# hangelwen/miR-PREFeR

Hardware: AMD Instinct MI355X
Metric: precursor windows folded+filtered/sec (L=300) (higher is better)
Workload: dtype int16/int32 (energies in 0.01 kcal/mol)

## Files before the change

mir-prefer_amd/csrc/fold_lds_kernel.hip:

```cpp
#include <algorithm>
#include "fold_lds_common.h"
#include "fold_ctl.h"
#ifndef MIRP_CPERIOD0
#define MIRP_CPERIOD0 0
#endif
#ifndef MIRP_CPERIOD1
#define MIRP_CPERIOD1 64
#endif
#define CPOOL_ROUNDS 4

namespace mirp {

template <int MODEL, bool SPARSE, int NT = LNT>
__global__ void __launch_bounds__(NT, 4) fold_lds_kernel(
    const FoldParams* __restrict__ P, const unsigned char* __restrict__ seqs, const long long* __restrict__ offs, const int* __restrict__ win_lens,
    int n_work, int win_base, int span, short* __restrict__ slabs, size_t slab_shorts, int* __restrict__ win_state,
    unsigned int* __restrict__ work_counter, int* __restrict__ fallback_list,
    unsigned int* __restrict__ fallback_count, int max_lines, int ss_stride, MirpFoldLine* __restrict__ out_lines, char* __restrict__ out_ss,
    int* __restrict__ out_nlines, int* __restrict__ out_mfe, int* __restrict__ out_status, int light_clocks_arg, long long* __restrict__ dbg_cycles_arg,
    const int* __restrict__ todo_list, const unsigned int* __restrict__ todo_count, int* __restrict__ dense_list, unsigned int* __restrict__ dense_count) {
#include "fold_lds_kernel_body.h"
}

template <int MODEL, bool SPARSE, int NT>
__device__ __forceinline__ void fold_lds_body(

    const FoldParams* __restrict__ P, const unsigned char* __restrict__ seqs, const long long* __restrict__ offs, const int* __restrict__ win_lens,
    int n_work, int win_base, int span, short* __restrict__ slabs, size_t slab_shorts, int* __restrict__ win_state,
    unsigned int* __restrict__ work_counter, int* __restrict__ fallback_list,
    unsigned int* __restrict__ fallback_count, int max_lines, int ss_stride, MirpFoldLine* __restrict__ out_lines, char* __restrict__ out_ss,
    int* __restrict__ out_nlines, int* __restrict__ out_mfe, int* __restrict__ out_status, int light_clocks_arg, long long* __restrict__ dbg_cycles_arg,
    const int* __restrict__ todo_list, const unsigned int* __restrict__ todo_count, int* __restrict__ dense_list, unsigned int* __restrict__ dense_count) {
#include "fold_lds_kernel_body.h"
}
#ifndef MIRP_FILL_TWO_ATTR
#define MIRP_FILL_TWO_ATTR __attribute__((amdgpu_num_vgpr(56)))
#endif
template <>
__global__ void MIRP_FILL_TWO_ATTR __launch_bounds__(LNT2, 4) fold_lds_kernel<0, true, LNT2>(

    const FoldParams* __restrict__ P, const unsigned char* __restrict__ seqs, const long long* __restrict__ offs, const int* __restrict__ win_lens,
    int n_work, int win_base, int span, short* __restrict__ slabs, size_t slab_shorts, int* __restrict__ win_state,
    unsigned int* __restrict__ work_counter, int* __restrict__ fallback_list,
    unsigned int* __restrict__ fallback_count, int max_lines, int ss_stride, MirpFoldLine* __restrict__ out_lines, char* __restrict__ out_ss,
    int* __restrict__ out_nlines, int* __restrict__ out_mfe, int* __restrict__ out_status, int light_clocks_arg, long long* __restrict__ dbg_cycles_arg,
    const int* __restrict__ todo_list, const unsigned int* __restrict__ todo_count, int* __restrict__ dense_list, unsigned int* __restrict__ dense_count) {
    fold_lds_body<0, true, LNT2>(P, seqs, offs, win_lens, n_work, win_base, span, slabs, slab_shorts, win_state, work_counter, fallback_list, fallback_count, max_lines, ss_stride, out_lines, out_ss, out_nlines, out_mfe, out_status, light_clocks_arg, dbg_cycles_arg, todo_list, todo_count, dense_list, dense_count);
}

#ifndef ENT
#define ENT 256
#endif
#ifndef MIRP_EPI_WGS
#define MIRP_EPI_WGS 8
#endif
__global__ void __launch_bounds__(ENT, MIRP_EPI_WGS) fold_lds_epilogue_kernel(
    const FoldParams* __restrict__ P, const unsigned char* __restrict__ seqs, const long long* __restrict__ offs, const int* __restrict__ win_lens,
    int n_work, int span, const short* __restrict__ slabs, size_t slab_shorts, const int* __restrict__ win_state, unsigned int* __restrict__ work_counter,
    int max_lines, int ss_stride, MirpFoldLine* __restrict__ out_lines, char* __restrict__ out_ss, int* __restrict__ out_nlines,
    int* __restrict__ out_mfe, int* __restrict__ out_status) {
    extern __shared__ __align__(16) unsigned char smem[];
    const int nc = LCAP + 8;
    int* f3 = (int*)smem;
    int* starts = f3 + nc;
    int* lens = starts + max_lines;
    int* btstk = lens + max_lines;
    int* misc = btstk + (ENT / 64) * 3 * BT_STACK;
    int* off = misc + 16;
    short* spec = (short*)(off + LDMAX + 2);
    unsigned char* S = (unsigned char*)(spec + 3 * nc);
    unsigned char* seq = S + nc;
    char* btbuf = (char*)(seq + nc);
    EpiTables* EP = (EpiTables*)(smem + ((((size_t)(btbuf - (char*)smem) + (ENT / 64) * nc) + 15) & ~(size_t)15));
    short* xtab = (short*)(EP + 1);
    unsigned char* pq2 = (unsigned char*)(xtab + XTAB_N);
    short* ppart = (short*)(pq2 + nc);
    const int tid = threadIdx.x;
    fill_epi_tables(EP, P, tid, ENT);
    fill_ext_table(xtab, P, tid, ENT);
    __syncthreads();
    EPI_INIT();
    for (;;) {
        if (tid == 0) misc[0] = (int)atomicAdd(work_counter, 1u);
        __syncthreads();
        const int win = misc[0];
        __syncthreads();
        if (win >= n_work) break;
        if (win_state[win] == 1) {
            const long long o0 = offs[win];
            const int n = win_lens ? win_lens[win] : (int)(offs[win + 1] - o0);
            const int D = (span - 1 < n - 1) ? span - 1 : n - 1;
            for (int x = tid; x <= n + 1; x += ENT) {
                unsigned char ch = 0;
                if (x >= 1 && x <= n) {
                    ch = seqs[o0 + x - 1];
                    if (ch >= 'a' && ch <= 'z') ch -= 32;
                    if (ch == 'T') ch = 'U';
                }
                seq[x] = ch;
                S[x] = ch == 'A' ? 1 : ch == 'C' ? 2 : ch == 'G' ? 3 : ch == 'U' ? 4 : 0;
            }
            if (tid < ARCH_RB) off[tid] = arch_rowblk_off(tid, n, span);
            __syncthreads();
            if (tid == 0) { S[0] = S[n]; S[n + 1] = S[1]; }
            for (int x = tid + 1; x <= n; x += ENT) pq2[x] = (unsigned char)((S[x] * 6 + (x < n ? (int)S[x + 1] : 5)) * 2);
            special_hairpins(P, seq, n, spec, nc, tid, ENT);
            __syncthreads();
            WinCtx X;
            X.P = P; X.S = S; X.seq = seq; X.f3 = f3; X.spec = spec; X.ldspec = nc; X.n = n; X.D = D; X.E = EP; X.xtab = xtab; X.pq2 = pq2; X.pp = ppart;
            LTab TB;
            TB.carch = slabs + (size_t)win * 3 * slab_shorts; TB.fml = TB.carch + slab_shorts; TB.off = off;
            TB.tb = reinterpret_cast<const unsigned short*>(TB.carch + 2 * slab_shorts);
            fold_epilogue<LTab, ENT>(X, TB, span, f3, starts, lens, btbuf, nc, btstk, misc + 8, win, max_lines, ss_stride, out_lines, out_ss, out_nlines,
                                    out_mfe, out_status);
        }
        __syncthreads();
    }
    EPI_FLUSH();
}

struct LTab185 {
    static constexpr bool kTiled = true;
    const short* carch;
    const short* fml;
    const unsigned short* tb;
    const int* off;
    int n, D, Dm;
    __device__ __forceinline__ int at(int d, int i) const { return off[(i - 1) >> 3] + ((i - 1) & 7) + 8 * (d - 4); }
    __device__ __forceinline__ int C(int i, int j) const {
        const int d = j - i;
        if (d <= TURN || d > D || i < 1 || j > n) return V_INF;
        const int v = carch[at(d, i)];
        return v == I16_INF ? V_INF : v;
    }
    __device__ __forceinline__ int Mm(int i, int j) const {
        const int d = j - i;
        if (d <= TURN || d > Dm || i < 1 || j > n) return V_INF;
        const int v = (unsigned short)fml[at(d, i)];
        return v == 65535 ? V_INF : v - FML_BIAS;
    }
    __device__ __forceinline__ int TB(int i, int j) const { return tb[at(j - i, i)]; }
};

#ifndef MIRP_EPI185_WGS
#define MIRP_EPI185_WGS 8
#endif
__global__ void __launch_bounds__(ENT, MIRP_EPI185_WGS) fold185_lds_epilogue_kernel(
    const FoldParams* __restrict__ P, const unsigned char* __restrict__ seqs, const long long* __restrict__ offs, const int* __restrict__ win_lens,
    int n_work, int span, const short* __restrict__ slabs, size_t slab_shorts, const int* __restrict__ win_state, unsigned int* __restrict__ work_counter,
    int max_lines, int ss_stride, MirpFoldLine* __restrict__ out_lines, char* __restrict__ out_ss, int* __restrict__ out_nlines,
    int* __restrict__ out_mfe, int* __restrict__ out_status) {
    extern __shared__ __align__(16) unsigned char smem[];
    const int nc = LCAP + 8;
    int* f3 = (int*)smem;
    int* starts = f3 + nc + 8;
    int* lens = starts + max_lines;
    int* btstk = lens + max_lines;
    int* red = btstk + (ENT / 64) * 3 * V_BT_STACK;
    int* misc = red + ENT / 64 + 8;
    int* off = misc + 4;
    short* tetra = (short*)(off + LDMAX + 2);
    unsigned char* S = (unsigned char*)(tetra + nc);
    unsigned char* seq = S + nc;
    char* btbuf = (char*)(seq + nc);
    short* dg = (short*)(smem + ((((size_t)(btbuf - (char*)smem) + (ENT / 64) * (nc + 8)) + 15) & ~(size_t)15));
    const int tid = threadIdx.x;
    if (tid < 40) { dg[tid] = (short)P->dangle5[tid / 5][tid % 5]; dg[40 + tid] = (short)P->dangle3[tid / 5][tid % 5]; }
    __syncthreads();
    EPI_INIT();
    for (;;) {
        if (tid == 0) misc[0] = (int)atomicAdd(work_counter, 1u);
        __syncthreads();
        const int win = misc[0];
        __syncthreads();
        if (win >= n_work) break;
        if (win_state[win] == 1) {
            const long long o0 = offs[win];
            const int n = win_lens ? win_lens[win] : (int)(offs[win + 1] - o0);
            for (int x = tid; x <= n + 1; x += ENT) {
                unsigned char ch = 0;
                if (x >= 1 && x <= n) {
                    ch = seqs[o0 + x - 1];
                    if (ch >= 'a' && ch <= 'z') ch -= 32;
                    if (ch == 'T') ch = 'U';
                }
                seq[x] = ch;
// ... 136 lines not shown
```

mir-prefer_amd/csrc/fold_lds_kernel_body.h:

```cpp
    extern __shared__ __align__(16) unsigned char smem[];
    constexpr bool TWO = NT != LNT;
    static_assert(NT == LNT || NT == LNT2, "workgroup size");
    constexpr int NW = NT / 64;
    constexpr LdsLayout LY = lds_layout<MODEL, SPARSE, TWO>();
#ifdef MIRP_DIAG
    const bool light = light_clocks_arg != 0;
    long long* const dbg_cycles = dbg_cycles_arg;
#else
    constexpr bool light = false;
    constexpr long long* dbg_cycles = nullptr;
    (void)light_clocks_arg; (void)dbg_cycles_arg;
#endif
    constexpr int DMLR = MODEL ? 5 : 3;
#define ENT_OUTER(mmo, mm1) ((unsigned)(((mmo) & 1023) | (((mm1) & 1023) << 10)))
    const int tau_s = __builtin_amdgcn_readfirstlane(P->TerminalAU);
    constexpr int GEN_WD = 5;
    long long tA = 0, tB = 0, tS = 0, tE = 0, t0 = 0;
    long long tR = 0, nR = 0, nB = 0;
    long long wB = 0, wA1 = 0, wA2 = 0, wW = 0, wt = 0;
    unsigned short* fml = (unsigned short*)(smem + LY.fml);
    unsigned short* cring = (unsigned short*)(smem + LY.aux);
    short* dmlring = (short*)(cring + CRING_ROWS * CSTR);
    int* acc = (int*)(dmlring + DMLR * LCAP);
    constexpr int NACC = SPARSE ? 6 : 5;
// ... 208 lines not shown
                }
                const int k0 = (NW - 1 - wave) * 64 + lane;
#pragma unroll
                for (int r = 0; r < A2_PRE; r++) {
                    const int k = k0 + r * NT;
                    if (k < lim) {
                        int i; bool ok;
                        (void)a2_entry(k, i, ok);
                        const unsigned sum = a2g[r] + (unsigned)poolB[k];
                        if (ok && sum < 65535u) atomicMin(&mdec[i], (int)sum - 2 * FML_BIAS);
                    }
                }
                for (int k = k0 + A2_PRE * NT; k < lim; k += NT) {
                    int i; bool ok;
                    const unsigned g = fml_g[a2_entry(k, i, ok)];
                    const unsigned sum = g + (unsigned)poolB[k];
                    if (ok && sum < 65535u) atomicMin(&mdec[i], (int)sum - 2 * FML_BIAS);
                }
                asm volatile("s_waitcnt lgkmcnt(0)" : "+v"(pnv) : : "memory");
                { const int pn = __builtin_amdgcn_readfirstlane(pnv); sp_snap = pn < pool_cap ? pn : pool_cap; }
            };
            auto splits_sparse185 = [&]() {
                const int lim = sp_snap;
                int pnv;
                {
                    const unsigned pa = (unsigned)(size_t)(__attribute__((address_space(3))) int*)&misc[3];
                    asm volatile("ds_read_b32 %0, %1" : "=v"(pnv) : "v"(pa) : "memory");
                }
                for (int k = (NW - 1 - wave) * 64 + lane; k < lim; k += NT) {
                    const unsigned lo = poolA[k], hi = poolB32[k];
                    const int p = (int)(lo & 511u), q = (int)((lo >> 9) & 511u);
                    const int valb = (int)(hi & 0xffffu), e5 = -(int)((hi >> 16) & 255u), e3 = -(int)(hi >> 24);
                    const int i0 = q - d, t0 = p - 1 - i0;
                    const int oA0 = 7 - 4 * n + (__mul24(t0, 2 * n + 1 - t0) >> 1) + ((t0 - 4 + (n & 1)) >> 1) + i0;
                    const int oA1 = oA0 - tri_len_any(t0 - 1, n);
                    const int oB1 = oA1 - tri_len_any(t0 - 2, n) + 1;
                    const bool c0 = i0 >= 1, c1 = i0 >= 0 && q + 1 <= n;
                    const bool vA0 = c0 && t0 >= TURN + 1, vA1 = c0 && t0 - 1 >= TURN + 1, vB0 = c1 && t0 - 1 >= TURN + 1, vB1 = c1 && t0 - 2 >= TURN + 1;
                    const int a0 = fml[vA0 ? oA0 : 1], a1 = fml[vA1 ? oA1 : 1], b0 = fml[vB0 ? oA1 + 1 : 1], b1 = fml[vB1 ? oB1 : 1];
                    int best0 = INF, best1 = INF;
                    if (vA0 && a0 != 65535) best0 = a0 + valb;
                    if (vA1 && a1 != 65535) { const int v = a1 + valb + e5; best0 = v < best0 ? v : best0; }
                    if (vB0 && b0 != 65535) best1 = b0 + valb + e3;
                    if (vB1 && b1 != 65535) { const int v = b1 + valb + e5 + e3; best1 = v < best1 ? v : best1; }
                    if (best0 < INF) atomicMin(&mdec[i0], best0 - 2 * FML_BIAS);
                    if (best1 < INF) atomicMin(&mdec[i0 + 1], best1 - 2 * FML_BIAS);
                }
                asm volatile("s_waitcnt lgkmcnt(0)" : "+v"(pnv) : : "memory");
                { const int pn = __builtin_amdgcn_readfirstlane(pnv); sp_snap = pn < pool_cap ? pn : pool_cap; }
            };
            auto splits_dense = [&]() {
                const int npair = (ncell + 1) >> 1;
                const int ncpad = (npair + 63) & ~63;
                if (ncpad != sp_ncpad) {
                    sp_ncpad = ncpad;
                    sp_nsub = (NT / ncpad) & ~1;
                    sp_pair = tid % ncpad;
                    sp_sub = __builtin_amdgcn_readfirstlane(tid / ncpad);
                    const int t0 = 4 + sp_sub, u0 = d - t0 - 1, s1 = sp_nsub;
                    sp_so1 = __builtin_amdgcn_readfirstlane(2 * tri_off(t0, n));
                    sp_si1 = __builtin_amdgcn_readfirstlane(2 * (tri_off(t0 + s1, n) - tri_off(t0, n)));
                    sp_so2 = __builtin_amdgcn_readfirstlane(2 * (tri_off(u0, n) + t0 + 1 - ((t0 & 1) ? 0 : 1)));
                    sp_si2 = __builtin_amdgcn_readfirstlane(2 * (tri_off(u0 - s1, n) - tri_off(u0, n) + s1));
                } else {
                    const int uprev = d - 1 - (4 + sp_sub) - 1;
                    sp_so2 += 2 * tri_len_any(uprev, n);
                    sp_si2 += 2 * sp_nsub;
                }
                const int nsub = sp_nsub, pair = sp_pair, sub = sp_sub;
                if (sub < nsub) {
                    const int i = 2 * pair + 1;
                    const int s1 = nsub;
                    int t = 4 + sub;
                    const int odd = t & 1;
                    int so1 = sp_so1, so2 = sp_so2, si1 = sp_si1, si2 = sp_si2;
                    const int sss = 2 * s1 * s1;
                    us2 bu = {65535, 65535};
                    typedef const __attribute__((address_space(3))) unsigned* lds_cu32;
                    const unsigned fb0 = (unsigned)(size_t)(lds_cu32)reinterpret_cast<const unsigned*>(fml + i);
                    unsigned va = fb0 + (unsigned)so1, vb = fb0 + (unsigned)so2;
#define MIRP_SSTEP() do { va += (unsigned)si1; vb += (unsigned)si2; asm volatile("s_sub_i32 %0, %0, %2\n\ts_sub_i32 %1, %1, %2" : "+s"(si1), "+s"(si2) : "s"(sss) : "scc"); } while (0)
#define MIRP_LDA() (*(lds_cu32)(va))
#define MIRP_LDB(o) (*(lds_cu32)(vb + (o)))
                    auto group = [&](auto ODD, auto KK) {
                        constexpr bool kOdd = decltype(ODD)::value;
                        constexpr int K = decltype(KK)::value;
                        unsigned a[K], b[K], c[K];
#pragma unroll
                        for (int k = 0; k < K; k++) {
                            a[k] = MIRP_LDA(); b[k] = MIRP_LDB(0);
                            if (!kOdd) c[k] = MIRP_LDB(4);
                            MIRP_SSTEP();
                        }
                        us2 e[K];
#pragma unroll
                        for (int k = 0; k < K; k++) {
                            const unsigned bw = kOdd ? b[k] : __builtin_amdgcn_alignbit(c[k], b[k], 16);
                            us2 av, bv;
                            __builtin_memcpy(&av, &a[k], 4); __builtin_memcpy(&bv, &bw, 4);
                            e[k] = __builtin_elementwise_add_sat(av, bv);
                        }
#pragma unroll
                        for (int w = 1; w < K; w *= 2)
#pragma unroll
                            for (int k = 0; k + w < K; k += 2 * w) e[k] = __builtin_elementwise_min(e[k], e[k + w]);
                        bu = __builtin_elementwise_min(bu, e[0]);
                        t += K * s1;
                    };
                    auto relax = [&](auto ODD) {
                        while (t + 7 * s1 <= d - 5) group(ODD, std::integral_constant<int, 8>{});
                        if (t + 3 * s1 <= d - 5) group(ODD, std::integral_constant<int, 4>{});
                        if (t + s1 <= d - 5) group(ODD, std::integral_constant<int, 2>{});
                        if (t <= d - 5) group(ODD, std::integral_constant<int, 1>{});
                    };
                    if (odd) relax(std::true_type{}); else relax(std::false_type{});
#undef MIRP_SSTEP
#undef MIRP_LDA
#undef MIRP_LDB
                    const unsigned r0 = bu[0], r1 = bu[1];
                    if (i <= ncell && r0 < 65535u) atomicMin(&mdec[i], (int)r0 - 2 * FML_BIAS);
                    if (i + 1 <= ncell && r1 < 65535u) atomicMin(&mdec[i + 1], (int)r1 - 2 * FML_BIAS);
                }
            };
            const bool swap_order = !SPARSE && (wave & 1);
            auto splits = [&]() { if constexpr (SPARSE && MODEL != 0) splits_sparse185(); else if constexpr (TWO) splits_sparse2(); else if constexpr (SPARSE) splits_sparse(); else splits_dense(); };
            if (swap_order) splits();
            if constexpr (TWO) a2_prefetch();
            if (dbg_cycles && lane == 0 && !light) wt = clock64();
            if (d >= 6 && d <= D) {
                const list_t* clist = list + (d % 3) * LSEG;
                const bool mix = d - 2 - (TURN + 1) >= MAXLOOP && d + 1 <= D;
                const int ncp = a1_ncp;
                const int done = a1_done;
                const int rem = ncp - done;
                const int nblk = (rem + 63) >> 6;
                int ncp2;
                if (lc_have) { asm volatile("s_waitcnt lgkmcnt(0)" : "+v"(lc_pre) : : "memory"); ncp2 = __builtin_amdgcn_readfirstlane(lc_pre); }
                else ncp2 = __builtin_amdgcn_readfirstlane(lcnt[(d + 1) % 6]);
                a1_ncp = ncp2;
                const int room = nblk * 64 - rem;
                const int take2 = mix ? (room < ncp2 ? room : ncp2) : 0;
                a1_done = take2;
                unsigned* ckey2 = reinterpret_cast<unsigned*>(acc + MIRP_CK(d + 1) * LCAP);
                unsigned aent = 0;
                {
                    const int ka = lane - (64 - room);
                    if (ka >= 0 && ka < take2) aent = list[((d + 1) % 3) * LSEG + ka];
                }
#define MIRP_XROWS15 9, 7
#define MIRP_XROWS8 8
#define MIRP_XROWS9 10
                A1 a;
                a.P = P; a.T = &T; a.S = S; a.cring = cring; a.pax = pax; a.qbr = qbr; a.code4 = code4; a.n = n;
#pragma nounroll
                for (int pass = 0; pass < (TWO ? 2 : 1); pass++) {
                const int role = TWO ? (wave < 4 ? wave + 8 * pass : wave < 6 ? (pass ? wave : wave + 10) : (pass ? wave : wave + 6))
                                     : wave < 4 ? wave : wave < 6 ? wave + 10 : wave < 12 ? wave + 2 : wave - 8;
                for (int blk = 0; blk < nblk; blk++) {
                    {
                        int r0 = d - 2, um = d - 2 - (TURN + 1) < MAXLOOP ? d - 2 - (TURN + 1) : MAXLOOP;
                        asm volatile("" : "+s"(r0), "+s"(um));
                        a.r0 = r0; a.um = um;
                        a.rowtab = P->ring_rowoff[r0 & 31];
                    }
                    const int k = blk * 64 + lane;
                    const bool own = k < rem, ahead = !own && aent != 0;
                    const bool act = own || ahead;
                    const unsigned ent = own ? clist[done + k] : ahead ? aent : (1u | (1u << 9));
                    const int i = ent & 511, type = (ent >> 9) & 7, j = i + d + (ahead ? 1 : 0);
                    a.cring = cring + (ahead ? CSTR : 0);
                    unsigned* ck = ahead ? ckey2 : ckey;
                    unsigned res = KEY_NONE;
                    int au1 = 0, mmo = 0, mm1 = 0;
                    if (role < 14 || MODEL == 0) {
                        au1 = type > 2 ? tau_s : 0;
                        mmo = ((int)(ent << 10)) >> 22; mm1 = ((int)ent) >> 22;
                    }
                    if (role < 8) {
#define MIRP_GEN(CK)                                                                      \
    switch (role) {                                                                       \
    case 0: res = MIRP_A1G<CK MIRP_A1WD, 30, 23>(a, i, j, mmo); if (CK) a1_i1<CK, 28, 29>(a, i, j, xi); else a1_i1f<28, 29>(a, i, j, xi); break;      \
    case 1: res = MIRP_A1G<CK MIRP_A1WD, 29, 24>(a, i, j, mmo); if (CK) a1_i1<CK, 25, 27>(a, i, j, xi); else a1_i1f<25, 27>(a, i, j, xi); break;      \
    case 2: res = MIRP_A1G<CK MIRP_A1WD, 28, 25>(a, i, j, mmo); if (CK) a1_i0<CK, 26, 29>(a, i, j, xi); else a1_i0f<26, 29>(a, i, j, xi); break;      \
    case 3: res = MIRP_A1G<CK MIRP_A1WD, 27, 26>(a, i, j, mmo); if (CK) a1_b1<CK, 26, 30>(a, i, j, xb); else a1_b1f<26, 30>(a, i, j, xb); break;      \
    case 4: res = MIRP_A1G<CK MIRP_A1WD, MIRP_ROWS4>(a, i, j, mmo); break;                    \
    case 5: res = MIRP_A1G<CK MIRP_A1WD, MIRP_ROWS5>(a, i, j, mmo); break;                    \
    case 6: res = MIRP_A1G<CK MIRP_A1WD, MIRP_ROWS6>(a, i, j, mmo); break;                    \
    default: res = MIRP_A1G<CK MIRP_A1WD, MIRP_ROWS7>(a, i, j, mmo); break;               \
    }
#define MIRP_XGEN(CK)                                                                     \
    switch (role) {                                                                       \
    case 15: rx = MIRP_A1G<CK MIRP_A1WD, MIRP_XROWS15>(a, i, j, mmo); break;                         \
    case 8: rx = MIRP_A1G<CK MIRP_A1WD, MIRP_XROWS8>(a, i, j, mmo); break;                           \
    case 9: rx = MIRP_A1G<CK MIRP_A1WD, MIRP_XROWS9>(a, i, j, mmo); break;                           \
    default: break;                                                                       \
    }
                        unsigned xb = KEY_INF, xi = KEY_INF;
                        if constexpr (MODEL == 0) {
#define MIRP_A1G a1_generic_w
#define MIRP_A1WD , GEN_WD
#define MIRP_ROWS4 22, 17, 12
#define MIRP_ROWS5 21, 18, 11
#define MIRP_ROWS6 20, 16, 13
#define MIRP_ROWS7 19, 15, 14, 6
                            if (RAMPF || a.um >= MAXLOOP) { MIRP_GEN(false) } else { MIRP_GEN(true) }
#undef MIRP_A1G
#undef MIRP_A1WD
#undef MIRP_ROWS4
#undef MIRP_ROWS5
#undef MIRP_ROWS6
#undef MIRP_ROWS7
                        } else {
#define MIRP_A1G a1_generic
#define MIRP_A1WD
#define MIRP_ROWS4 22, 17, 12, 7
#define MIRP_ROWS5 21, 18, 11, 8
#define MIRP_ROWS6 20, 16, 13, 9
#define MIRP_ROWS7 19, 15, 14, 10, 6
                            if (RAMPF || a.um >= MAXLOOP) { MIRP_GEN(false) } else { MIRP_GEN(true) }
#undef MIRP_A1G
#undef MIRP_A1WD
#undef MIRP_ROWS4
#undef MIRP_ROWS5
#undef MIRP_ROWS6
#undef MIRP_ROWS7
                        }
                        if (role < 4) {
                            const unsigned rb = a1_key(xb, -32768 - OTH_BIAS + au1);
                            const unsigned ri = a1_key(xi, -32768 - OTH_BIAS + mm1);
                            res = rb < res ? rb : res;
                            res = ri < res ? ri : res;
                        }
#undef MIRP_GEN
                    } else if (role < 14) {
                        unsigned bb = KEY_INF, bi = KEY_INF;
                        if (RAMPF || a.um >= MAXLOOP) {
                            switch (role) {
                            case 8: a1_b0f<2, 18>(a, i, j, bb); break;
                            case 9: a1_b0f<19, 30>(a, i, j, bb); a1_b1f<2, 6>(a, i, j, bb); break;
                            case 10: a1_b1f<7, 22>(a, i, j, bb); break;
                            case 11: a1_b1f<23, 25>(a, i, j, bb); a1_i0f<3, 15>(a, i, j, bi); break;
                            case 12: a1_i0f<16, 25>(a, i, j, bi); a1_i1f<3, 8>(a, i, j, bi); break;
                            default: a1_i1f<9, 24>(a, i, j, bi); break;
                            }
                        } else {
                            switch (role) {
                            case 8: a1_b0<true, 2, 18>(a, i, j, bb); break;
                            case 9: a1_b0<true, 19, 30>(a, i, j, bb); a1_b1<true, 2, 6>(a, i, j, bb); break;
                            case 10: a1_b1<true, 7, 22>(a, i, j, bb); break;
                            case 11: a1_b1<true, 23, 25>(a, i, j, bb); a1_i0<true, 3, 15>(a, i, j, bi); break;
                            case 12: a1_i0<true, 16, 25>(a, i, j, bi); a1_i1<true, 3, 8>(a, i, j, bi); break;
                            default: a1_i1<true, 9, 24>(a, i, j, bi); break;
                            }
                        }
                        const unsigned rb = a1_key(bb, -32768 - OTH_BIAS + au1);
                        const unsigned ri = a1_key(bi, -32768 - OTH_BIAS + mm1);
                        res = rb < ri ? rb : ri;
                    } else if (RAMPF || a.um >= MAXLOOP) {
                        res = role == 14 ? a1_small14f(a, i, j, type, ahead) : a1_small15f(a, i, j, type);
                    } else {
                        const int si1 = S[i + 1], sj1 = S[j - 1];
                        int ra, ca, rb2, cb2;
                        unsigned ka, kb2;
                        if (role == 14) {
                            a1_small_g<1, 1>(a, i, j, type, si1, sj1, ra, ca); a1_small_g<1, 2>(a, i, j, type, si1, sj1, rb2, cb2);
                            unsigned r00 = KEY_NONE;
                            a1_small<0, 0>(a, i, j, type, si1, sj1, r00); a1_small<0, 1>(a, i, j, type, si1, sj1, res); a1_small<1, 0>(a, i, j, type, si1, sj1, res);
                            if (!ahead) res = r00 < res ? r00 : res;
                            ka = 1 << 5 | 1; kb2 = 1 << 5 | 2;
                        } else {
                            a1_small_g<2, 1>(a, i, j, type, si1, sj1, ra, ca); a1_small_g<2, 2>(a, i, j, type, si1, sj1, rb2, cb2);
                            a1_small<2, 3>(a, i, j, type, si1, sj1, res); a1_small<3, 2>(a, i, j, type, si1, sj1, res);
                            ka = 2 << 5 | 1; kb2 = 2 << 5 | 2;
                        }
                        if (ca < INF) { const unsigned k = ((unsigned)(ra + ca + KEY_BIAS) << 10) | ka; res = k < res ? k : res; }
                        if (cb2 < INF) { const unsigned k = ((unsigned)(rb2 + cb2 + KEY_BIAS) << 10) | kb2; res = k < res ? k : res; }
                    }
                    if constexpr (MODEL == 0) {
                        if (role >= 8) {
                            unsigned rx = KEY_NONE;
#define MIRP_A1G a1_generic_w
#define MIRP_A1WD , GEN_WD
                            if (RAMPF || a.um >= MAXLOOP) { MIRP_XGEN(false) } else { MIRP_XGEN(true) }
#undef MIRP_A1G
#undef MIRP_A1WD
                            res = rx < res ? rx : res;
                        }
                    }
                    if (act && res != KEY_NONE) atomicMin(&ck[i], res);
                }
                if (role == 14 && done > 0) {
                    const bool act = lane < done;
                    const unsigned ent = act ? clist[lane] : (1u | (1u << 9));
                    const int i = ent & 511, type = (ent >> 9) & 7, j = i + d;
                    int r0 = d - 2, um = MAXLOOP;
                    asm volatile("" : "+s"(r0), "+s"(um));
                    a.r0 = r0; a.um = um; a.cring = cring;
                    unsigned res = KEY_NONE;
                    a1_small<0, 0>(a, i, j, type, S[i + 1], S[j - 1], res);
                    if (act && res != KEY_NONE) atomicMin(&ckey[i], res);
                }
                }
                if (dbg_cycles && lane == 0 && wave == 9 && !light) {
                    const int b = nblk < 3 ? nblk : 3;
                    atomicAdd((unsigned long long*)&dbg_cycles[68 + b], (unsigned long long)(clock64() - wt));
                    atomicAdd((unsigned long long*)&dbg_cycles[72 + b], 1ull);
                }
            }
            if (dbg_cycles && lane == 0 && !light) { const long long t = clock64(); wA1 += t - wt; wt = t; }
            if (!swap_order) splits();
        };
        auto phaseB0 = [&](const int d) {
            const int ncell = n - d;
            unsigned* ckey = reinterpret_cast<unsigned*>(acc + MIRP_CK(d) * LCAP);
            int* mdec = mdec_of(d);
            int cbase = 0, cand = 0; unsigned cent = 0, cval = 0;
            unsigned long long cbal = 0;
            const int hp_u = P->hairpinE[d - 1 < MIRP_HP_MAX ? d - 1 : MIRP_HP_MAX - 1];
            const int od = TWO ? (d & 1) * FRING_STR : tri_off(d, n), od1 = TWO ? ((d - 1) & 1) * FRING_STR : tri_off(d - 1, n);
            const int x = tid;
            int lt = 0, lbase = 0, loi = 0, ent_terms = 0;
            unsigned long long lbal = 0;
            const bool do_list = d + 3 <= D;
            if (tid == 0) lcnt[(d + 4) % 6] = 0;
            if (x < ncell) {
                const int i = x + 1, j = i + d, u = d - 1;
                lds_vu8 Sv = (lds_vu8)S;
                const int s_im1 = pb_si & 7, s_i = (pb_si >> 3) & 7, s_ip1 = (pb_si >> 6) & 7, s_jm1 = pb_sj & 7, s_j = (pb_sj >> 3) & 7, s_jp1 = (pb_sj >> 6) & 7;
                const int s_j2 = (pb_sj >> 9) & 7, s_j3 = (pb_sj >> 12) & 7;
                pb_sj = (pb_sj >> 3) | (((int)Sv[j + 4] & 7) << 12);
                int md = mdec[i];
                if constexpr (SPARSE) { md = dml_carry < md ? dml_carry : md; dml_carry = md; }
                const unsigned kk = ckey[i];
                const int dmlv = dmlring[((d + DMLR - 2) % DMLR) * LCAP + i + 1];
                int fa = 65535, fb = 65535;
                if (d > 4) { fa = fml[od1 + i]; fb = fml[od1 + i + 1]; }
                int sv = -32768;
                if (u == 4) sv = spec[nc + i]; else if (u == 6) sv = spec[2 * nc + i]; else if (u == 3) sv = spec[i];
                if (do_list) {
                    if (j + 3 <= n) { lt = pair_type(s_i, s_j3); loi = lt * 25 + s_ip1 * 5 + s_j2; }
                    lbal = __ballot(lt != 0);
                    if (lbal && lane == 0) {
                        const unsigned la = (unsigned)(size_t)(__attribute__((address_space(3))) int*)&lcnt[(d + 3) % 6];
                        asm volatile("ds_add_rtn_u32 %0, %1, %2" : "=v"(lbase) : "v"(la), "v"((int)__popcll(lbal)) : "memory");
                    }
                }
                const int type = pair_type(s_i, s_j);
                const int rt = rtype_of(type);
                const int tau = T.TerminalAU, mli = T.ML_intern, mlc = T.ML_closing;
                const int mmH = T.mismatchH[type * 25 + s_ip1 * 5 + s_jm1];
                const int mmMc = T.mismatchM[rt * 25 + s_jm1 * 5 + s_ip1];
                const int mmMs = T.mismatchM[type * 25 + s_im1 * 5 + s_jp1];
                const int dg5 = T.dangle5[type * 5 + s_im1], dg3 = T.dangle3[type * 5 + s_jp1];
                const int mmI = T.mismatchI[rt * 25 + s_jp1 * 5 + s_im1];
                ent_terms = ENT_OUTER((int)T.mismatchI[loi], (int)T.mismatch1nI[loi]);
                const int au = type > 2 ? tau : 0;
                int cv = INF, tb = 0;
                if (type) {
                    const int cint = kk == KEY_NONE ? INF : (int)(kk >> 10) - KEY_BIAS;
                    int h;
                    if (sv != -32768) h = sv;
                    else if (u == 3) h = hp_u + au;
                    else h = hp_u + mmH;
                    cv = h < cint ? h : cint;
                    if (dmlv != I16_INF) {
                        const int e = dmlv + mlc + mli + (rt > 2 ? tau : 0) + mmMc;
                        cv = e < cv ? e : cv;
                    }
                    if (cint < INF && cint == cv && h != cv) tb = (int)(kk & 1023u) + 1;
                }
                int m = INF;
                {
                    const int a = fa == 65535 ? INF : fa - FML_BIAS, b = fb == 65535 ? INF : fb - FML_BIAS;
                    m = a < b ? a : b;
                }
                if (type) {
                    const int stem = mli + au + ((i > 1 && j < n) ? mmMs : (i > 1) ? dg5 : (j < n) ? dg3 : 0);
                    const int e = cv + stem;
                    if constexpr (SPARSE) cand = cv < INF && e < m && e < md;
                    m = e < m ? e : m;
                }
                m = md < m ? md : m;
                if constexpr (SPARSE) {
                    cbal = __ballot(cand != 0);
                    if (cbal && lane == 0) {
                        const unsigned pa = (unsigned)(size_t)(__attribute__((address_space(3))) int*)&misc[3];
                        asm volatile("ds_add_rtn_u32 %0, %1, %2" : "=v"(cbase) : "v"(pa), "v"((int)__popcll(cbal)) : "memory");
                    }
                    cent = (unsigned)(i - 1) | ((unsigned)j << 9);
                }
                if ((cv < INF && (cv > FIN_LIMIT || cv < -FIN_LIMIT)) || (m < INF && (m > FML_MAX || m < -FML_BIAS)) ||
                    (md < INF && (md > FIN_LIMIT || md < -FIN_LIMIT))) misc[1] = 1;
                const short c16 = cv >= INF ? (short)I16_INF : (short)cv;
                const unsigned short m16 = m >= INF ? (unsigned short)65535 : (unsigned short)(m + FML_BIAS);
                const unsigned short g16 = cv < INF ? (unsigned short)(cv + mmI + 32768) : (unsigned short)65535;
                cring[(d & 31) * CSTR + i] = g16;
                if ((d & 31) == 0) cring[32 * CSTR + i] = g16;
                carch[abase + 8 * d] = c16;
                tb_out[abase + 8 * d] = (unsigned short)tb;
                fml[od + i] = m16;
                if constexpr (TWO) fml_out[abase + 8 * d] = (short)m16;
                dmlring[(d % DMLR) * LCAP + i] = md >= INF ? (short)I16_INF : (short)md;
                ckey[i] = KEY_NONE;
                if constexpr (SPARSE) { mdec_of(d + 2)[i] = INF; cval = m16; }
                else mdec[i] = INF;
            }
            if constexpr (SPARSE) {
                if (cbal) {
                    asm volatile("s_waitcnt lgkmcnt(0)" : "+v"(cbase) : : "memory");
                    const int at = __builtin_amdgcn_readfirstlane(cbase) + (int)__popcll(cbal & ((1ull << lane) - 1ull));
                    if (cand) {
                        if (at < pool_cap) { poolA[at] = cent; poolB[at] = (unsigned short)cval; }
                        else misc[2] = 1;
                    }
                }
            }
            asm volatile("s_waitcnt lgkmcnt(0)" : "+v"(lbase) : : "memory");
            const int lb = __builtin_amdgcn_readfirstlane(lbase);
            if (lt) list[(d % 3) * LSEG + lb + __popcll(lbal & ((1ull << lane) - 1ull))] = (list_t)((unsigned)(x + 1) | ((unsigned)lt << 9) | ((unsigned)ent_terms << 12));
        };
        auto phaseB1 = [&](const int d) {
            const int ncell = n - d;
            unsigned* ckey = reinterpret_cast<unsigned*>(acc + MIRP_CK(d) * LCAP);
            int* mdec = mdec_of(d);
            int cand = 0; unsigned cent = 0, cval = 0;
            if constexpr (SPARSE) { if (tid < 11) pbits[((d + 1) & 3) * 11 + tid] = 0; }
            const int hp_u = P->hairpinE[d - 1 < MIRP_HP_MAX ? d - 1 : MIRP_HP_MAX - 1];
            const int od = tri_off(d, n), od1 = tri_off(d - 1, n);
            const int x = tid;
            int lt = 0, lbase = 0, loi = 0, ent_terms = 0;
            unsigned long long lbal = 0;
            const bool do_list = d + 3 <= D;
            const bool has1 = d - 1 >= 4, has2 = d - 2 >= 4;
            if (tid == 0) lcnt[(d + 4) % 6] = 0;
            if (x < ncell) {
                const int i = x + 1, j = i + d, u = d - 1;
                lds_vu8 Sv = (lds_vu8)S;
                const int s_im1 = pb_si & 7, s_i = (pb_si >> 3) & 7, s_ip1 = (pb_si >> 6) & 7, s_jm1 = pb_sj & 7, s_j = (pb_sj >> 3) & 7, s_jp1 = (pb_sj >> 6) & 7;
                const int s_j2 = (pb_sj >> 9) & 7, s_j3 = (pb_sj >> 12) & 7;
                pb_sj = (pb_sj >> 3) | ((int)Sv[j + 4] << 12);
                int md = mdec[i];
                if constexpr (SPARSE) { md = dml_carry < md ? dml_carry : md; dml_carry = md; }
                const unsigned kk = ckey[i];
                const int q11 = dmlring[((d + DMLR - 2) % DMLR) * LCAP + i + 1], q21 = dmlring[((d + DMLR - 3) % DMLR) * LCAP + i + 2];
                const int q12 = dmlring[((d + DMLR - 3) % DMLR) * LCAP + i + 1], q22 = dmlring[((d + DMLR - 4) % DMLR) * LCAP + i + 2];
                int fa = 65535, fb = 65535;
                if (d > 4) { fa = fml[od1 + i]; fb = fml[od1 + i + 1]; }
                const int tetra = u == 4 ? (int)spec[nc + i] : 0;
                const unsigned g1 = has1 ? (unsigned)cring[((d - 1) & 31) * CSTR + i + 1] : 65535u;
                const unsigned g2 = has1 ? (unsigned)cring[((d - 1) & 31) * CSTR + i] : 65535u;
                const unsigned g3 = has2 ? (unsigned)cring[((d - 2) & 31) * CSTR + i + 1] : 65535u;
                if (do_list) {
                    if (j + 3 <= n) { lt = pair_type(s_i, s_j3); loi = lt * 25 + s_ip1 * 5 + s_j2; }
                    lbal = __ballot(lt != 0);
                    if (lbal && lane == 0) {
                        const unsigned la = (unsigned)(size_t)(__attribute__((address_space(3))) int*)&lcnt[(d + 3) % 6];
                        asm volatile("ds_add_rtn_u32 %0, %1, %2" : "=v"(lbase) : "v"(la), "v"((int)__popcll(lbal)) : "memory");
                    }
                }
                const int type = d > D ? 0 : pair_type(s_i, s_j);
                const int rt = rtype_of(type);
                const int tp1 = pair_type(s_ip1, s_j), tp2 = pair_type(s_i, s_jm1), tp3 = pair_type(s_ip1, s_jm1);
                const int tau = T.TerminalAU, mli = T.ML_intern, mlc = T.ML_closing;
                const int mmH = T.mismatchH[type * 25 + s_ip1 * 5 + s_jm1];
                const int e3 = T.dangle3[rt * 5 + s_ip1], e5 = T.dangle5[rt * 5 + s_jm1];
                const int mmI = T.mismatchI[rt * 25 + s_jp1 * 5 + s_im1];
// ... 194 lines not shown
```

Before: 368,000.

## Fuse A1 two-pass role loop into per-block loop and skip idle phaseB waves

```diff
diff --git a/mir-prefer_amd/csrc/fold_lds_kernel.hip b/mir-prefer_amd/csrc/fold_lds_kernel.hip
--- a/mir-prefer_amd/csrc/fold_lds_kernel.hip
+++ b/mir-prefer_amd/csrc/fold_lds_kernel.hip
@@ -8,6 +8,12 @@
 #define MIRP_CPERIOD1 64
 #endif
 #define CPOOL_ROUNDS 4
+#ifndef MIRP_A1_FUSE
+#define MIRP_A1_FUSE 1
+#endif
+#ifndef MIRP_PHASEB_SKIP
+#define MIRP_PHASEB_SKIP 1
+#endif
 
 namespace mirp {
 
@@ -31,7 +37,11 @@
     unsigned int* __restrict__ fallback_count, int max_lines, int ss_stride, MirpFoldLine* __restrict__ out_lines, char* __restrict__ out_ss,
     int* __restrict__ out_nlines, int* __restrict__ out_mfe, int* __restrict__ out_status, int light_clocks_arg, long long* __restrict__ dbg_cycles_arg,
     const int* __restrict__ todo_list, const unsigned int* __restrict__ todo_count, int* __restrict__ dense_list, unsigned int* __restrict__ dense_count) {
+#if MIRP_A1_FUSE
+#define MIRP_A1_FUSED
+#endif
 #include "fold_lds_kernel_body.h"
+#undef MIRP_A1_FUSED
 }
 #ifndef MIRP_FILL_TWO_ATTR
 #define MIRP_FILL_TWO_ATTR __attribute__((amdgpu_num_vgpr(56)))
diff --git a/mir-prefer_amd/csrc/fold_lds_kernel_body.h b/mir-prefer_amd/csrc/fold_lds_kernel_body.h
--- a/mir-prefer_amd/csrc/fold_lds_kernel_body.h
+++ b/mir-prefer_amd/csrc/fold_lds_kernel_body.h
@@ -384,21 +384,37 @@
 #define MIRP_XROWS9 10
                 A1 a;
                 a.P = P; a.T = &T; a.S = S; a.cring = cring; a.pax = pax; a.qbr = qbr; a.code4 = code4; a.n = n;
+#define MIRP_A1_BLOCK()                                                                                                        \
+                    {                                                                                                          \
+                        int r0 = d - 2, um = d - 2 - (TURN + 1) < MAXLOOP ? d - 2 - (TURN + 1) : MAXLOOP;                      \
+                        asm volatile("" : "+s"(r0), "+s"(um));                                                                 \
+                        a.r0 = r0; a.um = um;                                                                                  \
+                        a.rowtab = P->ring_rowoff[r0 & 31];                                                                    \
+                    }                                                                                                          \
+                    const int k = blk * 64 + lane;                                                                             \
+                    const bool own = k < rem, ahead = !own && aent != 0;          \
+                    const bool act = own || ahead;                                                                             \
+                    unsigned ent = own ? clist[done + k] : ahead ? aent : (1u | (1u << 9));
+#ifdef MIRP_A1_FUSED
+                const int role1st = wave < 4 ? wave : wave < 6 ? wave + 10 : wave + 6, role2nd = wave < 4 ? wave + 8 : wave;
+                for (int blk = 0; blk < nblk; blk++) {
+                    MIRP_A1_BLOCK()
+                    unsigned best = KEY_NONE;
+                    int npass = 2;
+                    asm volatile("" : "+s"(npass));
+                    for (int pass = 0; pass < npass; pass++) {
+                    const int role = pass ? role2nd : role1st;
+                    asm volatile("" : "+v"(ent));
+#define MIRP_A1_ROLE14_HERE (wave == 4)
+#else
 #pragma nounroll
                 for (int pass = 0; pass < (TWO ? 2 : 1); pass++) {
                 const int role = TWO ? (wave < 4 ? wave + 8 * pass : wave < 6 ? (pass ? wave : wave + 10) : (pass ? wave : wave + 6))
                                      : wave < 4 ? wave : wave < 6 ? wave + 10 : wave < 12 ? wave + 2 : wave - 8;
                 for (int blk = 0; blk < nblk; blk++) {
-                    {
-                        int r0 = d - 2, um = d - 2 - (TURN + 1) < MAXLOOP ? d - 2 - (TURN + 1) : MAXLOOP;
-                        asm volatile("" : "+s"(r0), "+s"(um));
-                        a.r0 = r0; a.um = um;
-                        a.rowtab = P->ring_rowoff[r0 & 31];
-                    }
-                    const int k = blk * 64 + lane;
-                    const bool own = k < rem, ahead = !own && aent != 0;
-                    const bool act = own || ahead;
-                    const unsigned ent = own ? clist[done + k] : ahead ? aent : (1u | (1u << 9));
+                    MIRP_A1_BLOCK()
+#define MIRP_A1_ROLE14_HERE (role == 14)
+#endif
                     const int i = ent & 511, type = (ent >> 9) & 7, j = i + d + (ahead ? 1 : 0);
                     a.cring = cring + (ahead ? CSTR : 0);
                     unsigned* ck = ahead ? ckey2 : ckey;
@@ -519,9 +535,16 @@
                             res = rx < res ? rx : res;
                         }
                     }
+#ifdef MIRP_A1_FUSED
+                    best = res < best ? res : best;
+                    }
+                    if (act && best != KEY_NONE) atomicMin(&(ahead ? ckey2 : ckey)[ent & 511], best);
+                }
+#else
                     if (act && res != KEY_NONE) atomicMin(&ck[i], res);
                 }
-                if (role == 14 && done > 0) {
+#endif
+                if (MIRP_A1_ROLE14_HERE && done > 0) {
                     const bool act = lane < done;
                     const unsigned ent = act ? clist[lane] : (1u | (1u << 9));
                     const int i = ent & 511, type = (ent >> 9) & 7, j = i + d;
@@ -532,7 +555,11 @@
                     a1_small<0, 0>(a, i, j, type, S[i + 1], S[j - 1], res);
                     if (act && res != KEY_NONE) atomicMin(&ckey[i], res);
                 }
-                }
+#ifndef MIRP_A1_FUSED
+                }
+#endif
+#undef MIRP_A1_ROLE14_HERE
+#undef MIRP_A1_BLOCK
                 if (dbg_cycles && lane == 0 && wave == 9 && !light) {
                     const int b = nblk < 3 ? nblk : 3;
                     atomicAdd((unsigned long long*)&dbg_cycles[68 + b], (unsigned long long)(clock64() - wt));
@@ -544,6 +571,7 @@
         };
         auto phaseB0 = [&](const int d) {
             const int ncell = n - d;
+            if constexpr (TWO && MIRP_PHASEB_SKIP) { if (wave * 64 >= ncell) return; }
             unsigned* ckey = reinterpret_cast<unsigned*>(acc + MIRP_CK(d) * LCAP);
             int* mdec = mdec_of(d);
             int cbase = 0, cand = 0; unsigned cent = 0, cval = 0;
```

New measurement: 397,700, median of 6. 1.08x the previous value.
